# ChicyChen/LOCO-Edit

Measured on AMD Instinct MI355X. Metric: edit-directions/sec (top-5 PMP-Jacobian SVD @256^2) + vT cos-sim vs ref, higher is better.
Workload: dtype bf16x3 (split-bf16 MFMA operands, fp32 accumulate + fp32 storage); 1 GPU; CelebA-HQ DDPM 256x256 top-5 local basis (l_eye-sized mask, L=2400), t=0.6T, 12 power iterations, one GPU; multi_gpu_form=single, probes_total=5, probes_per_gpu=5, kept=5, n_iter=12, mask_L=2400, weights=synthetic seed 0, streams=2

## Files before the change

loco-edit_amd/csrc/conv_bf16_kernel.h:

```cpp
#pragma once
#include "kernels.h"
#include <cstdlib>
#include <type_traits>

namespace loco {


typedef float f32x16 __attribute__((ext_vector_type(16)));
typedef float f32x4 __attribute__((ext_vector_type(4)));
typedef f32x4 f32x4_u __attribute__((aligned(4)));
typedef float f32x2 __attribute__((ext_vector_type(2)));
typedef f32x2 f32x2_u __attribute__((aligned(4)));
typedef __bf16 bf16x8 __attribute__((ext_vector_type(8)));
typedef _Float16 f16x8 __attribute__((ext_vector_type(8)));
typedef short s16x8 __attribute__((ext_vector_type(8)));

enum : int { PR_BF16X3 = 0, PR_F16 = 1 };

constexpr int BKC = 16;
constexpr bool LIVE_MASK = true;
constexpr bool EARLY_W = true;
constexpr int NDUMMY = 8;

__device__ __forceinline__ float sigmoidf2_(float y) { return __builtin_amdgcn_rcpf(1.0f + __expf(-y)); }
// ... 608 lines not shown
            have = hi < nsg4 * nhy2 && sg < nseg && hy < halo_h;
            if (!have) v_q4 = 0;
        } else if (tid < 4 * per_q) {
            int rem;
            idivmod_small(tid, per_q, v_q4, rem);
            idivmod_small(rem, nseg, hy, sg);
            have = true;
        }
        if (have) {
            int Y = oy0 - a.pad + hy, X0 = ox0 - a.pad + 4 * sg;
            bool rowok = (Y >= 0 && Y < a.Hin);
            v_pos0 = hy * halo_w + 4 * sg;
            v_cnt = halo_w - 4 * sg < 4 ? halo_w - 4 * sg : 4;
            v_voff = rowok ? Y * a.Win + X0 : 0;
#pragma unroll
            for (int pxi = 0; pxi < 4; ++pxi)
                if (rowok && X0 + pxi >= 0 && X0 + pxi < a.Win && pxi < v_cnt) v_pm |= 1u << pxi;
        }
#pragma unroll
        for (int pxi = 0; pxi < 4; ++pxi)
            v_rec[pxi] = (v_pos0 >= 0 && pxi < v_cnt) ? v_pos0 + pxi : halo_sz + (tid & (NDUMMY - 1));
        v_goff = (unsigned)(((long)v_q4 * 4 * in_plane + v_voff + 16) * 4);
    }

    int hoff[TN];
#pragma unroll
    for (int j = 0; j < TN; ++j) {
        int p = (wn * TN + j) * 32 + l31;
        int ty, tx;
        idivmod_small(p, TW, ty, tx);
        hoff[j] = ty * S * halo_w + tx * S;
    }
    int hbyte[TN];
#pragma unroll
    for (int j = 0; j < TN; ++j) hbyte[j] = hrec_off<PR>(hoff[j], khalf);
    int aoff_hi[TM], aoff_lo[TM];
#pragma unroll
    for (int i = 0; i < TM; ++i) {
        int p = (wm * TM + i) * 32 + l31;
        aoff_hi[i] = rec_off<PR>(p, khalf);
        aoff_lo[i] = PR == PR_F16 ? 0 : rec_off<PR>(p, 2 + khalf);
    }

    if constexpr (PHASE != 2) {
#pragma unroll
        for (int i = 0; i < TM; ++i)
#pragma unroll
            for (int j = 0; j < TN; ++j)
#pragma unroll
                for (int r = 0; r < 16; ++r) acc[i][j][r] = 0.0f;
    }

    const int nchunks = (a.Cin + BKC - 1) / BKC;
    const int cps = __builtin_amdgcn_readfirstlane((nchunks + a.nsplit - 1) / a.nsplit);
    const int cbeg = split * cps;
    const int cend = (cbeg + cps < nchunks) ? cbeg + cps : nchunks;

    const float* inb = a.in + (long)b * a.in_bs;
    const float2* sxb = NEEDP ? a.sx : nullptr;
    const float* scb = (MODE == CM_GN_SILU || MODE == CM_GN || MODE == CM_GN_GELU) ? a.sc + (long)b * a.scsh_bs : nullptr;
    const float* shb = (MODE == CM_GN_SILU || MODE == CM_GN || MODE == CM_GN_GELU) ? a.sh + (long)b * a.scsh_bs : nullptr;
    const int wpitch = (a.Cout + 31) & ~31;
    const uint4* wg = reinterpret_cast<const uint4*>(a.wb);

    float hv[NITEM][8];
    float2 pv[NEEDP ? NITEM : 1][8];
    float cA[(MODE == CM_NONE) ? 1 : 16], cB[(MODE == CM_NONE) ? 1 : 16];
    const float* tcb = NEEDP ? a.tc + (long)b * a.tc_bs : nullptr;

    constexpr int NPART = (!GEN && NROW >= 2) ? 2 : 1;
    constexpr int KP = 4 / NPART;
    struct HaloRegs {
        f32x4 dq[GEN ? 1 : KP];
        f32x4 sq[(!GEN && NEEDP) ? KP : 1][2];
        f32x4 cq[(!GEN && MODE != CM_NONE) ? (KP == 4 ? 2 : 1) : 1];
    };
    auto cq_a = [&](const HaloRegs& R, int kk) -> float {
        if constexpr (GEN || MODE == CM_NONE) return 0.f;
        else if constexpr (NEEDP) { if constexpr (KP == 4) return R.cq[kk >> 1][(kk & 1) * 2]; else return R.cq[0][kk * 2]; }
        else return R.cq[0][kk];
    };
    auto cq_b = [&](const HaloRegs& R, int kk) -> float {
        if constexpr (GEN || MODE == CM_NONE) return 0.f;
        else if constexpr (NEEDP) { if constexpr (KP == 4) return R.cq[kk >> 1][(kk & 1) * 2 + 1]; else return R.cq[0][kk * 2 + 1]; }
        else if constexpr (KP == 4) return R.cq[1][kk];
        else return R.cq[0][2 + kk];
    };
    HaloRegs hr;
    bool pf_live = true, dma_live = true;
#ifdef LOCO_DUAL_STAMP
    const bool wi_halo = (a.no_deep & 2) != 0, wi_dma = (a.no_deep & 4) != 0, wi_novalu = (a.no_deep & 8) != 0;
#endif
    auto prefetch_hv = [&](HaloRegs& R, int chunk, int part) {
        const unsigned cb = (unsigned)chunk * ((unsigned)(BKC * 4) * (unsigned)in_plane);
        const char* pk = reinterpret_cast<const char*>(inb - 16) + cb;
        const char* sk = reinterpret_cast<const char*>(reinterpret_cast<const float*>(sxb) - 32) + 2u * cb;
        const unsigned pl = (unsigned)in_plane * 4u;
#pragma unroll
        for (int kk = 0; kk < KP; ++kk) {
#ifdef LOCO_DUAL_STAMP
            const unsigned po = (pf_live && !wi_halo) ? v_goff + (unsigned)(part * KP + kk) * pl : 64u;
#else
            const unsigned po = pf_live ? v_goff + (unsigned)(part * KP + kk) * pl : 64u;
#endif
            R.dq[kk] = *reinterpret_cast<const f32x4_u*>(pk + po);
            if constexpr (NEEDP) {
                R.sq[kk][0] = *reinterpret_cast<const f32x4_u*>(sk + 2u * po);
                R.sq[kk][1] = *reinterpret_cast<const f32x4_u*>(sk + 2u * po + 16);
            }
        }
        const int c0 = chunk * BKC + v_q4 * 4 + part * KP;
        if constexpr (MODE != CM_NONE) {
            if constexpr (NEEDP) {
                R.cq[0] = *reinterpret_cast<const f32x4_u*>(tcb + 2 * c0);
                if constexpr (KP == 4) R.cq[1] = *reinterpret_cast<const f32x4_u*>(tcb + 2 * c0 + 4);
            } else if constexpr (KP == 4) {
                R.cq[0] = *reinterpret_cast<const f32x4_u*>(scb + c0);
                R.cq[1] = *reinterpret_cast<const f32x4_u*>(shb + c0);
// ... 9 lines not shown
#endif
        const int oct = v_q4 >> 1, half = v_q4 & 1;
#pragma unroll
        for (int pxi = 0; pxi < 4; ++pxi) {
            float r[KP];
#pragma unroll
            for (int kk = 0; kk < KP; ++kk) {
                float d = R.dq[kk][pxi];
                float v = d;
                if constexpr (MODE == CM_GN_SILU) {
                    float y = fmaf(cq_a(R, kk), d, cq_b(R, kk));
                    v = y * sigmoidf2_(y);
                } else if constexpr (MODE == CM_GN_GELU) {
                    v = act_fwd(fmaf(cq_a(R, kk), d, cq_b(R, kk)), ACT_GELU);
                } else if constexpr (MODE == CM_GN) {
                    v = fmaf(cq_a(R, kk), d, cq_b(R, kk));
                } else if constexpr (NEEDP) {
                    const float Sv = R.sq[kk][pxi >> 1][(pxi & 1) * 2], xh = R.sq[kk][pxi >> 1][(pxi & 1) * 2 + 1];
                    if constexpr (MODE == CM_TAN_SILU) v = Sv * fmaf(-xh, cq_b(R, kk), d - cq_a(R, kk));
                    else v = fmaf(-xh, cq_b(R, kk), fmaf(Sv, d, -cq_a(R, kk)));
                }
                r[kk] = ((v_pm >> pxi) & 1u) ? v : 0.0f;
            }
            unsigned char* dst = Hs + hrec_off<PR>(v_rec[pxi], oct) + half * 8 + part * (KP * 2);
            if constexpr (KP == 4) {
                uint2 h, l;
                cvt2<PR>(r[0], r[1], h.x, l.x);
                cvt2<PR>(r[2], r[3], h.y, l.y);
                *reinterpret_cast<uint2*>(dst) = h;
                if constexpr (PR == PR_BF16X3) *reinterpret_cast<uint2*>(dst + 32) = l;
            } else {
                unsigned h, l;
                cvt2<PR>(r[0], r[1], h, l);
                *reinterpret_cast<unsigned*>(dst) = h;
                if constexpr (PR == PR_BF16X3) *reinterpret_cast<unsigned*>(dst + 32) = l;
            }
        }
    };
    auto load_consts = [&](int chunk) {
        const int c0 = chunk * BKC;
        if constexpr (MODE != CM_NONE) {
#pragma unroll
            for (int kk = 0; kk < 16; ++kk) {
                int c = c0 + kk < a.Cin ? c0 + kk : a.Cin - 1;
                if constexpr (NEEDP) { cA[kk] = tcb[2 * c]; cB[kk] = tcb[2 * c + 1]; }
                else { cA[kk] = scb[c]; cB[kk] = shb[c]; }
            }
        }
    };
    auto load_regs = [&](float (&hvd)[NITEM][8], int chunk) {
        int c0 = chunk * BKC;
        long poff = 0;
        if constexpr (PIN) {
            const int cpp = a.Cin >> 6, ph = __builtin_amdgcn_readfirstlane(idiv_small(chunk, cpp));
            c0 = (chunk - ph * cpp) * BKC;
            poff = (long)(ph >> 1) * 2 * a.Win + (ph & 1);
        }
        if (PIN || c0 + BKC <= a.Cin) {
            if constexpr (TAPS == 9 && !NEEDP) {
                const unsigned lm = pf_live ? 0xffffffffu : 0u;
                const long pb4 = in_plane * 4;
                const unsigned char* pk = reinterpret_cast<const unsigned char*>(inb) + (long)c0 * pb4;
#pragma unroll
                for (int k = 0; k < 8; ++k) {
#pragma unroll
                    for (int i = 0; i < NITEM; ++i) hvd[i][k] = *reinterpret_cast<const float*>(pk + ((ivoff[i] * 4u) & lm));
                    pk += pb4;
                }
            } else {
#pragma unroll
            for (int k = 0; k < 8; ++k) {
                const float* pk = inb + (long)(c0 + k) * in_plane + poff;
                const float2* sk = NEEDP ? sxb + (long)(c0 + k) * in_plane : nullptr;
#pragma unroll
                for (int i = 0; i < NITEM; ++i) {
                    hvd[i][k] = pk[pf_live ? ivoff[i] : 0u];
                    if constexpr (NEEDP) pv[i][k] = sk[pf_live ? ivoff[i] : 0u];
                }
            }
            }
        } else {
#pragma unroll
            for (int i = 0; i < NITEM; ++i) {
#pragma unroll
                for (int k = 0; k < 8; ++k) {
                    int c = c0 + ioct[i] * 8 + k;
                    int cc = c < a.Cin ? c : a.Cin - 1;
                    unsigned vo = ivoff[i] - (unsigned)(ioct[i] * 8 * (int)in_plane);
                    float v = inb[(long)cc * in_plane + vo];
                    hvd[i][k] = c < a.Cin ? v : 0.0f;
                    if constexpr (NEEDP) {
                        float2 pp = sxb[(long)cc * in_plane + vo];
                        pv[i][k] = c < a.Cin ? pp : make_float2(0.f, 0.f);
                    }
                }
            }
        }
    };
    auto prefetch_h = [&](int chunk, int part) {
        if constexpr (!GEN) { prefetch_hv(hr, chunk, part); return; }
        load_consts(chunk);
        load_regs(hv, chunk);
    };
    unsigned wrel[NWV];
#pragma unroll
    for (int i = 0; i < NWV; ++i) {
        int e = tid + i * NTHR;
        if (e >= WTOT) e = WTOT - 1;
        int tap = e / (MT * NPC), rem = e - tap * (MT * NPC);
        int rec = co0 + rem / NPC;
        if (rec >= wpitch) rec = wpitch - 1;
        wrel[i] = (unsigned)((tap * wpitch + rec) * NPC + (rem % NPC)) * 16u;
    }
    typedef __attribute__((address_space(3))) unsigned char lds_u8;
    typedef const __attribute__((address_space(1))) unsigned char glb_u8;
    auto dma_w = [&](int chunk, int row, unsigned char* Wdst) {
        const unsigned char* wbase = reinterpret_cast<const unsigned char*>(wg) +
                                     (unsigned)(chunk * TAPS + row * NTS) * ((unsigned)wpitch * (unsigned)RB);
#pragma unroll
        for (int i = 0; i < NWV; ++i) {
            const int e0 = (wave * 64 + i * NTHR);
            if ((WTOT % NTHR) == 0 || e0 < WTOT)
#ifdef LOCO_DUAL_STAMP
                __builtin_amdgcn_global_load_lds((glb_u8*)(wbase + ((dma_live && !wi_dma) ? wrel[i] : 0u)), (lds_u8*)(Wdst + e0 * 16), 16, 0, 0);
#else
                __builtin_amdgcn_global_load_lds((glb_u8*)(wbase + (dma_live ? wrel[i] : 0u)), (lds_u8*)(Wdst + e0 * 16), 16, 0, 0);
#endif
        }
    };
    auto stage_regs = [&](const float (&hvs)[NITEM][8], int chunk, unsigned char* Hd, auto whole_tag) {
        constexpr bool WHOLE = decltype(whole_tag)::value;
        const int c0 = chunk * BKC;
#pragma unroll
        for (int i = 0; i < NITEM; ++i) {
            if (ipos[i] < 0) continue;
            float v[8];
#pragma unroll
            for (int k = 0; k < 8; ++k) {
                int c = c0 + ioct[i] * 8 + k;
                float r = 0.0f;
                if (ival[i] && (WHOLE || c < a.Cin)) {
                    float d = hvs[i][k];
                    if constexpr (MODE == CM_NONE) {
                        r = d;
                    } else {
                        const float ca = ioct[i] ? cA[8 + k] : cA[k];
                        const float cb = ioct[i] ? cB[8 + k] : cB[k];
                        if constexpr (MODE == CM_GN_SILU) {
                            float y = fmaf(ca, d, cb);
                            r = y * sigmoidf2_(y);
                        } else if constexpr (MODE == CM_GN_GELU) {
                            r = act_fwd(fmaf(ca, d, cb), ACT_GELU);
                        } else if constexpr (MODE == CM_GN) {
                            r = fmaf(ca, d, cb);
                        } else {
                            float Sv = pv[i][k].x, xh = pv[i][k].y;
                            if constexpr (MODE == CM_TAN_SILU) r = Sv * fmaf(-xh, cb, d - ca);
                            else r = fmaf(-xh, cb, fmaf(Sv, d, -ca));
                        }
                    }
                }
                v[k] = r;
            }
            uint4 hi, lo;
            split8<PR>(v, hi, lo);
            *reinterpret_cast<uint4*>(Hd + hrec_off<PR>(ipos[i], ioct[i])) = hi;
            if constexpr (PR == PR_BF16X3) *reinterpret_cast<uint4*>(Hd + hrec_off<PR>(ipos[i], 2 + ioct[i])) = lo;
        }
    };
    auto stage_h = [&](int chunk, int part) {
        if constexpr (!GEN) { stage_hv(hr, part); return; }
        stage_regs(hv, chunk, Hs, std::false_type{});
    };

    constexpr int NLO = PR == PR_BF16X3 ? 1 : 0;
    struct Frag { s16x8 ah[TM], al[NLO ? TM : 1], bh[TN], bl[NLO ? TN : 1]; };
    auto load_frag = [&](Frag& f, int row, int tp) {
        const int tapoff = (TAPS == 9) ? row * halo_w + tp : (TAPS == 4 ? tap0 + row * halo_w + tp : 0);
#pragma unroll
        for (int i = 0; i < TM; ++i) {
            f.ah[i] = *reinterpret_cast<const s16x8*>(Ws + tp * MT * RB + aoff_hi[i]);
#if defined(LOCO_WI_NOLO)
            if constexpr (NLO) f.al[i] = f.ah[i];
#else
            if constexpr (NLO) f.al[i] = *reinterpret_cast<const s16x8*>(Ws + tp * MT * RB + aoff_lo[i]);
#endif
        }
#pragma unroll
        for (int j = 0; j < TN; ++j) {
            const unsigned char* hp = Hs + tapoff * HP + hbyte[j];
            f.bh[j] = *reinterpret_cast<const s16x8*>(hp);
#if defined(LOCO_WI_NOLO)
            if constexpr (NLO) f.bl[j] = f.bh[j];
#else
            if constexpr (NLO) f.bl[j] = *reinterpret_cast<const s16x8*>(hp + 32);
#endif
        }
    };
    auto mma_frag = [&](const Frag& f) {
#pragma unroll
        for (int i = 0; i < TM; ++i)
#pragma unroll
            for (int j = 0; j < TN; ++j) {
                if constexpr (PR == PR_F16) {
                    acc[i][j] = __builtin_amdgcn_mfma_f32_32x32x16_f16(__builtin_bit_cast(f16x8, f.ah[i]),
                                                                       __builtin_bit_cast(f16x8, f.bh[j]), acc[i][j], 0, 0, 0);
                } else {
                    const bf16x8 ah = __builtin_bit_cast(bf16x8, f.ah[i]), al = __builtin_bit_cast(bf16x8, f.al[i]);
                    const bf16x8 bh = __builtin_bit_cast(bf16x8, f.bh[j]), bl = __builtin_bit_cast(bf16x8, f.bl[j]);
                    acc[i][j] = __builtin_amdgcn_mfma_f32_32x32x16_bf16(al, bh, acc[i][j], 0, 0, 0);
                    acc[i][j] = __builtin_amdgcn_mfma_f32_32x32x16_bf16(ah, bl, acc[i][j], 0, 0, 0);
                    acc[i][j] = __builtin_amdgcn_mfma_f32_32x32x16_bf16(ah, bh, acc[i][j], 0, 0, 0);
                }
            }
    };

    auto mma_one = [&](const Frag& f, int i, int j) {
        if constexpr (PR == PR_F16) {
            acc[i][j] = __builtin_amdgcn_mfma_f32_32x32x16_f16(__builtin_bit_cast(f16x8, f.ah[i]),
                                                               __builtin_bit_cast(f16x8, f.bh[j]), acc[i][j], 0, 0, 0);
        } else {
            const bf16x8 ah = __builtin_bit_cast(bf16x8, f.ah[i]), al = __builtin_bit_cast(bf16x8, f.al[i]);
            const bf16x8 bh = __builtin_bit_cast(bf16x8, f.bh[j]), bl = __builtin_bit_cast(bf16x8, f.bl[j]);
#if defined(LOCO_WI_MFMA16)
// ... 188 lines not shown
            issue(S3{}, cbeg + 3);
            commit(S0{}, cbeg, Hsb, Wsb);
            issue(S0{}, cbeg + 4);
            stage_end();
        }
        auto body = [&](auto stag, const int ci) {
            const int chunk = cbeg + ci;
            unsigned char* const Wcur = Wsb + (ci & 1) * WBYTES;
            unsigned char* const Wnxt = Wsb + ((ci + 1) & 1) * WBYTES;
            unsigned char* const Hcur = Hsb + (ci & 1) * HBYTES;
            unsigned char* const Hnxt = Hsb + ((ci + 1) & 1) * HBYTES;
            Ws = Wcur; Hs = Hcur;
            Frag f0;
            load_frag(f0, 0, 0);
            __builtin_amdgcn_sched_barrier(0);
            mma_frag(f0);
            commit(stag, cclamp(chunk + 1), Hnxt, Wnxt);
            issue(stag, chunk + 1 + D);
            stage_end();
        };
        int ci = 0;
        for (; ci + D <= nch; ci += D) {
            body(S1{}, ci); body(S2{}, ci + 1); body(S3{}, ci + 2); body(S0{}, ci + 3);
        }
        if (ci < nch) body(S1{}, ci);
        if (ci + 1 < nch) body(S2{}, ci + 1);
        if (ci + 2 < nch) body(S3{}, ci + 2);
      }
    }
    if (!deep_done) {
    if (nch > 0) {
        dma_w(cbeg, 0, Wsb);
        Hs = Hsb;
        if constexpr (!GEN && NPART == 2) {
            HaloRegs hr2;
            prefetch_hv(hr, cbeg, 0);
            prefetch_hv(hr2, cbeg, 1);
            stage_hv(hr, 0);
            stage_hv(hr2, 1);
        } else {
#pragma unroll
            for (int part = 0; part < NPART; ++part) {
                prefetch_h(cbeg, part);
                stage_h(cbeg, part);
            }
        }
        asm volatile("s_waitcnt vmcnt(0)" ::: "memory");
        if (NROW == 1 || NPART == 2) prefetch_h(cclamp(cbeg + 1), 0);
        stage_end();
    }
    for (int ci = 0; ci < nch; ++ci) {
        const int chunk = cbeg + ci;
        if constexpr (PIN) {
            const int ph = __builtin_amdgcn_readfirstlane(idiv_small(chunk, a.Cin >> 6));
            tap0 = (1 - (ph >> 1)) * halo_w + 1 - (ph & 1);
        }
#pragma unroll
        for (int row = 0; row < NROW; ++row) {
            const int s_ = ci * NROW + row;
            unsigned char* const Wcur = Wsb + (s_ & 1) * WBYTES;
            unsigned char* const Wnxt = Wsb + ((s_ + 1) & 1) * WBYTES;
            unsigned char* const Hcur = Hsb + (ci & 1) * HBYTES;
            unsigned char* const Hnxt = Hsb + ((ci + 1) & 1) * HBYTES;
            constexpr bool one = (NROW == 1);
            const int st_part = one ? 0 : (NPART == 2 ? (row == 0 ? 0 : row == 1 ? 1 : -1) : (row == NROW - 1 ? 0 : -1));
            const int ld_part = one ? 0 : (NPART == 2 ? (row == 0 ? 1 : row == 1 ? 0 : -1) : (row == 0 ? 0 : -1));
            const int ld_chunk = one ? chunk + 2 : ((NPART == 2 && row == 1) ? chunk + 2 : chunk + 1);
            constexpr bool MIDLOAD = !GEN;
            constexpr int NLD = KP + (NEEDP ? 2 * KP + 1 : (MODE != CM_NONE ? 2 : 0));
            {
                const int r1 = (row + 1) % NROW, dc = (row + 1) / NROW;
                dma_live = LIVE_MASK ? (chunk + dc <= clast) : true;
                dma_w(cclamp(chunk + dc), r1, Wnxt);
                dma_live = true;
            }
            Ws = Wcur; Hs = Hcur;
            Frag f0, f1;
            load_frag(f0, row, 0);
            if (NTS > 1) load_frag(f1, row, 1);
            __builtin_amdgcn_sched_barrier(0);
            mma_frag(f0);
            __builtin_amdgcn_sched_barrier(0);
            if (NTS > 2) load_frag(f0, row, 2);
            __builtin_amdgcn_sched_barrier(0);
            if (NTS > 1) mma_frag(f1);
            if (st_part >= 0) { Hs = Hnxt; stage_h(cclamp(chunk + 1), st_part); Hs = Hcur; }
            if (MIDLOAD && ld_part >= 0) { pf_live = LIVE_MASK ? (ld_chunk <= clast) : true; prefetch_h(cclamp(ld_chunk), ld_part); pf_live = true; }
            if (NTS > 2) mma_frag(f0);
            __builtin_amdgcn_sched_barrier(0);
            if (MIDLOAD && ld_part >= 0) {
                asm volatile("s_waitcnt vmcnt(%0)" :: "n"(NLD) : "memory");
            } else {
                asm volatile("s_waitcnt vmcnt(0)" ::: "memory");
                if (!MIDLOAD && ld_part >= 0) { pf_live = LIVE_MASK ? (ld_chunk <= clast) : true; prefetch_h(cclamp(ld_chunk), ld_part); pf_live = true; }
            }
            stage_end();
        }
    }
    }

    }

    if constexpr (PHASE == 1) {
        asm volatile("s_waitcnt lgkmcnt(0)" ::: "memory");
        __builtin_amdgcn_s_barrier();
        return;
    }
    LP_STAMP(3);
    if constexpr (POLY) conv_lowp_epilogue_poly<WM, WN, TM, TN>(a, acc, smem_b, cot_id, pa_, oy0, ox0, TW, tile_id, b);
    else conv_lowp_epilogue<WM, WN, TM, TN, (TAPS == 1 && PHASE == 0) ? (EPI_COT1 | EPI_STATS) : EPI_STATS>(a, acc, smem_b, co0, oy0, ox0, TW, tile_id, b, split);
    LP_STAMP(4);
#undef LP_STAMP
}

constexpr int lowp_min_waves(int taps, int nthr) { return (taps == 1 && nthr <= 256) ? 2 : 1; }
template <int TAPS, int WM, int WN, int TM, int TN, int MODE, int STG>
__global__ __launch_bounds__(WM * WN * 64, lowp_min_waves(TAPS, WM * WN * 64)) void conv_mfma_bf16x3(ConvArgs a) {
    f32x16 acc[TM][TN];
    conv_lowp_body<PR_BF16X3, TAPS, WM, WN, TM, TN, MODE, STG>(a, acc);
}
// ... 34 lines not shown
    if (lds > 64 * 1024) {
        static DeviceOnce once;
        if (first_on_device(once)) {
            (void)hipFuncSetAttribute(reinterpret_cast<const void*>(kern), hipFuncAttributeMaxDynamicSharedMemorySize,
                                      160 * 1024);
        }
    }
    hipLaunchKernelGGL(kern, grid, dim3(WM * WN * 64), lds, st, a);
}

template <int PR, int TAPS, int WM, int WN, int TM, int TN, int MODE>
static void launch_one_b(const ConvArgs& a, hipStream_t st) {
    const bool general = a.stride != 1 || a.upsample || a.zins || (a.Cin % BKC) != 0 || !a.in_padded;
    if constexpr (MODE == CM_NONE) {
        if (a.stride == 2) launch_one_b2<PR, TAPS, WM, WN, TM, TN, MODE, 2>(a, st);
        else if (TAPS == 9 && !general) launch_one_b2<PR, TAPS, WM, WN, TM, TN, MODE, 0>(a, st);
        else launch_one_b2<PR, TAPS, WM, WN, TM, TN, MODE, 1>(a, st);
        return;
    }
    if constexpr (MODE == CM_GN_SILU || MODE == CM_TAN_SILU || MODE == CM_GN_GELU) {
        if (general) { launch_one_b2<PR, TAPS, WM, WN, TM, TN, MODE, 1>(a, st); return; }
    }
    launch_one_b2<PR, TAPS, WM, WN, TM, TN, MODE, 0>(a, st);
}


template <int PR, int MODE>
void launch_kcat_b(const ConvArgs& a, hipStream_t st) {
    constexpr int WM = 2, WN = 4, TM = 2, TN = 2, MT = 128, NT = 256;
    const int TW = a.Wout < 32 ? a.Wout : 32, TH = NT / TW;
    size_t lds = (size_t)3 * 3 * MT * rec_bytes<PR>() + 2 * ((size_t)(TW + 2) * (TH + 2) + NDUMMY) * halo_pitch<PR>();
    dim3 grid(((a.Hout * a.Wout) / NT) * ((a.Cout + MT - 1) / MT) * a.B * a.nsplit);
    void (*kern)(ConvArgs);
    if constexpr (PR == PR_F16) kern = &conv_kcat_f16<WM, WN, TM, TN, MODE>;
    else kern = &conv_kcat_bf16x3<WM, WN, TM, TN, MODE>;
    static DeviceOnce once;
    if (first_on_device(once))
        (void)hipFuncSetAttribute(reinterpret_cast<const void*>(kern), hipFuncAttributeMaxDynamicSharedMemorySize, 160 * 1024);
    hipLaunchKernelGGL(kern, grid, dim3(WM * WN * 64), lds, st, a);
}

template <int PR>
void launch_poly_b(const ConvArgs& a, hipStream_t st) {
    ConvArgs v = a;
    v.Cout = 4 * a.Cout; v.Hout = a.Hin; v.Wout = a.Win;
    v.upsample = 0; v.zins = 0; v.stride = 1; v.pad = 1; v.nsplit = 1;
    launch_one_b2<PR, 4, 2, 4, 2, 2, CM_NONE, 0>(v, st);
}

template <int PR>
void launch_poly_in_b(const ConvArgs& a, hipStream_t st) {
    ConvArgs v = a;
    v.Cin = 4 * a.Cin; v.Hin = a.Hin / 2; v.Win = a.Win / 2;
    v.upsample = 0; v.zins = 0; v.stride = 1; v.pad = 1; v.nsplit = 1;
    launch_one_b2<PR, 4, 2, 4, 2, 2, CM_NONE, 1>(v, st);
}

template <int PR, int TAPS, int MODE>
void launch_tile_b(const ConvArgs& a, hipStream_t st) {
    switch (a.tile) {
        case 5:
            launch_one_b<PR, TAPS, 2, 4, 2, 2, MODE>(a, st);
            break;
        case 0: launch_one_b<PR, TAPS, 2, 2, 2, 2, MODE>(a, st); break;
        case 1: launch_one_b<PR, TAPS, 4, 1, 1, 2, MODE>(a, st); break;
        case 2: launch_one_b<PR, TAPS, 1, 4, 1, 1, MODE>(a, st); break;
        default: launch_one_b<PR, TAPS, 2, 2, 1, 1, MODE>(a, st); break;
    }
}


}
```

loco-edit_amd/csrc/conv_plan.hip:

```cpp
#include "kernels.h"
#include <cstdio>
#include <cstdlib>

namespace loco {

constexpr int BKC = 16;
constexpr int BKF = 8;

static const int kMT[6] = {128, 128, 32, 64, 128, 128}, kNT[6] = {128, 64, 128, 64, 256, 256};

static int env_int(const char* name, int dflt) {
    const char* e = getenv(name);
    return e ? atoi(e) : dflt;
}
static int pick_tile(int Cout, int HW) {
    if (HW >= 128) return Cout > 32 ? 0 : 2;
    return Cout > 64 ? 1 : 3;
}

static int conv_pick_nsplit(int Cin, int Cout, int Hout, int Wout, int B) {
    const int t = pick_tile(Cout, Hout * Wout);
    long blocks = (long)((Hout * Wout) / kNT[t]) * ((Cout + kMT[t] - 1) / kMT[t]) * B;
    int nchunks = (Cin + BKF - 1) / BKF;
    if (blocks >= 384 || nchunks < 8) return 1;
    int want = (int)((512 + blocks - 1) / blocks);
    int maxs = nchunks / 4;
    if (want > maxs) want = maxs;
    if (want > 32) want = 32;
    return want < 1 ? 1 : want;
}

static int conv_bf16_pick_tile(int Cout, int HW, int B, int tile_override) {
    if (B <= 1 && HW <= 1024 && HW >= 64 && (Cout % 64) == 0) return 3;
    int t = pick_tile(Cout, HW);
    if (t == 0 && HW >= 256) {
        if (tile_override >= 0) return tile_override;
        return 5;
    }
    return t;
}

constexpr int kTile0MaxHW = 65536;

static int bf16_tile_of(const ConvArgs& a, int tile_override = -1) {
    int tile = conv_bf16_pick_tile(a.Cout, a.Hout * a.Wout, a.B, tile_override);
    if (tile == 4) tile = 5;
    if (tile == 5 && a.taps == 1 && !a.gemm && a.B >= 2 && a.Hout * a.Wout <= kTile0MaxHW) return 0;
    if (a.stride == 2 && tile == 5) tile = 0;
    return tile;
}
static int tile_for(const ConvArgs& a, int prec, int tile_override) {
    return prec ? bf16_tile_of(a, tile_override) : pick_tile(a.Cout, a.Hout * a.Wout);
}
static int conv_bf16_tile_pixels(const ConvArgs& a) { return a.poly == 1 ? 512 : a.gemm ? 256 : kNT[a.tile]; }
int conv_bf16_tile_couts(const ConvArgs& a) { return a.gemm ? 64 * a.gemm_tm : kMT[a.tile]; }

static bool conv_poly_ok(const ConvEnv& e, const ConvArgs& a, int taps) {
    static const bool on = env_int("LOCO_POLYPHASE", 1) != 0;
    if (!on || e.prec < 1 || taps != 9 || a.mode != CM_NONE || !(a.upsample || a.zins) || a.stride != 1) return false;
    if (!(e.prec == 2 ? a.wph : a.wpb) || !a.in_padded || a.res || a.Cin2 > 0 || a.cot_d) return false;
    if (a.upsample ? a.pad != 1 : (a.pad != 1 && a.pad != 2)) return false;
    if ((a.Cin % BKC) != 0 || (a.Cout % 128) != 0 || a.B < 2) return false;
    if (a.Hin * a.Win < 4096 || a.Win < 32 || (a.Win % 32) != 0 || (a.Hin % 8) != 0) return false;
    return a.Hout == 2 * a.Hin && a.Wout == 2 * a.Win;
}
static bool conv_poly_in_ok(const ConvEnv& e, const ConvArgs& a, int taps) {
    static const bool on = env_int("LOCO_POLYPHASE", 1) != 0;
    if (!on || e.prec < 1 || taps != 9 || a.mode != CM_NONE || !a.pool2 || a.upsample || a.zins || a.stride != 1 || a.pad != 1) return false;
    if (!(e.prec == 2 ? a.wqh : a.wqb) || a.res || a.bias2 || a.Cin2 > 0 || a.cot_d) return false;
    if ((a.Cin % BKC) != 0 || (a.Cout % 128) != 0 || a.B < 2 || ((a.Hin | a.Win) & 1)) return false;
    if (a.Hout * a.Wout < 4096 || a.Wout < 32 || (a.Wout % 32) != 0 || (a.Hout % 8) != 0) return false;
    return a.Hin == 2 * a.Hout && a.Win == 2 * a.Wout;
}

static int conv_bf16_pick_nsplit(int Cin, int Cout, int Hout, int Wout, int B, int chip_share, int taps, int lanes) {
    const int HW = Hout * Wout;
    int t = conv_bf16_pick_tile(Cout, HW, B, -1);
    if (t == 4) t = 5;
    if (taps == 1 && t == 5 && B >= 2 && HW <= kTile0MaxHW) t = 0;
    long blocks = (long)(HW / kNT[t]) * ((Cout + kMT[t] - 1) / kMT[t]) * B;
    int nchunks = (Cin + BKC - 1) / BKC;
    int target = chip_share > 1 ? 256 / chip_share : (lanes == 2 ? 240 : 256);
    if (target < 32) target = 32;
    if (blocks >= target / 2 || nchunks < 8) return 1;
    int want = (int)(target / blocks);
    int maxs = nchunks / 4;
    if (want > maxs) want = maxs;
    if (want > 32) want = 32;
    return want < 1 ? 1 : want;
}

static bool conv_lowp_can_kcat(const ConvArgs& a) {
    static const bool on = env_int("LOCO_KCAT", 1) != 0;
    return on && a.Cin2 > 0 && a.nsplit == 1 && bf16_tile_of(a) == 5 && a.stride == 1 && !a.upsample && !a.zins && a.pad == 1 &&
           (a.Cin % BKC) == 0 && (a.Cin2 % BKC) == 0 && a.in_padded &&
           (a.mode == CM_GN_SILU || a.mode == CM_GN_GELU || a.mode == CM_TAN_SILU);
}
static bool conv_lowp_can_fuse_stats(const ConvArgs& a) {
    return a.nsplit <= 1 && !a.gemm && (a.Cout % conv_bf16_tile_couts(a)) == 0;
}

static bool conv_pair_ok(const ConvArgs& a) {
    static const bool on = env_int("LOCO_CONV_PAIR", 1) != 0;
    if (!on || a.poly || a.Hout * a.Wout < 16384 || a.taps != 9 || a.Cin2 > 0 || a.nsplit != 1 || a.stride != 1 || a.upsample || a.zins ||
        a.pad != 1 || !a.in_padded || (a.Cin % (2 * BKC)) != 0 || (a.Cout % 128) != 0 || (a.Wout % 32) != 0 || (a.Hout % 8) != 0)
        return false;
    if (!(a.mode == CM_NONE || a.mode == CM_GN_SILU || a.mode == CM_TAN_SILU || a.mode == CM_COT_SILU)) return false;
    return a.tile == 5;
}

static ConvArgs conv_shift_batch(const ConvArgs& a, int nb) {
    ConvArgs t = a;
    t.B = a.B - nb;
    t.in += (long)nb * a.in_bs; t.out += (long)nb * a.out_bs;
    if (t.prim) t.prim += (long)nb * a.prim_bs;
    if (t.bias2) t.bias2 += (long)nb * a.bias2_bs;
    if (t.res) t.res += (long)nb * a.res_bs;
    if (t.sc) { t.sc += (long)nb * a.scsh_bs; t.sh += (long)nb * a.scsh_bs; }
    if (t.mr) t.mr += (long)nb * a.mr_bs;
    if (t.tst) t.tst += (long)nb * a.tst_bs;
    if (t.tc) t.tc += (long)nb * a.tc_bs;
    if (t.in2) t.in2 += (long)nb * a.in2_bs;
    if (t.cot_d) { t.cot_d += (long)nb * a.cot_d_bs; t.cot_tc += (long)nb * a.cot_tc_bs; }
    if (t.st_part) t.st_part += (long)nb * a.Cout * ((a.Hout * a.Wout) / conv_bf16_tile_pixels(a)) * 2;
// ... 54 lines not shown
    while (s > 1 && nchunks / s < 4) --s;
    const size_t one = (size_t)(r / per_probe) * a.Cout * a.Hout * a.Wout;
    while (s > 1 && (size_t)s * one > partial_floats) --s;
    *split = s;
    return s > 1 ? (int)(r / per_probe) : 0;
}

static int stats_route(const ConvEnv& e, const StatAsk* q, bool want, ConvArgs& x, int s0, int B, int* keep_ntile) {
    if (!q || q->kind == ST_NONE) return SR_NONE;
    const int alone = q->norm ? SR_ALONE : SR_NONE;
    if (!want) return alone;
    if (x.nsplit > 1) return !q->norm ? SR_NONE : ((x.Hout * x.Wout) % 4 == 0 ? SR_SPLITK : SR_ALONE);
    const int ntile = (x.Hout * x.Wout) / conv_bf16_tile_pixels(x);
    const size_t need = (size_t)x.B * x.Cout * ntile * 2;
    const int epi = q->norm ? SR_EPI : SR_KEEP;
    const bool kept = q->keep && s0 == 0 && x.B == B && need <= q->keep_floats;
    if (q->kind == ST_FWD && x.poly != 1 && conv_lowp_can_fuse_stats(x) && (kept || (q->norm && need <= e.stpart_floats))) {
        x.st_part = kept ? q->keep : e.stpart; x.st_kind = ST_FWD;
        if (kept) *keep_ntile = ntile;
        return epi;
    }
    const bool cot_cache = q->kind == ST_COT && q->norm && q->sx && x.poly != 1;
    if ((q->kind == ST_TAN || cot_cache) && e.fuse_lin && !x.cot_d && conv_lowp_can_fuse_stats(x)) {
        const size_t lane_off = (size_t)e.lane_s0 * (q->keep_floats / e.max_batch);
        const bool keptl = q->kind == ST_TAN && q->keep && s0 == 0 && x.B == B && lane_off + need <= q->keep_floats;
        if (keptl || (q->norm && need <= e.stpart_floats)) {
            x.st_part = keptl ? q->keep + lane_off : e.stpart; x.st_kind = q->kind; x.st_x = q->prim;
            if (q->kind == ST_COT) x.st_sx = q->sx;
            if (keptl) *keep_ntile = ntile;
            return epi;
        }
    }
    return alone;
}

static ConvLaunch plan_launch(const ConvEnv& e, const StatAsk* q, bool want, const ConvArgs& x, int s0, int B, int* keep_ntile) {
    ConvLaunch l;
    l.args = x;
    l.s0 = s0;
    l.args.tile = tile_for(x, e.prec, -1);
    l.stats = stats_route(e, q, want, l.args, s0, B, keep_ntile);
    if (l.stats == SR_EPI || l.stats == SR_KEEP) l.ntile = (x.Hout * x.Wout) / conv_bf16_tile_pixels(l.args);
    conv_plan_tile_pair(l.args, e.prec, -1);
    return l;
}

ConvPlan plan_conv(const ConvEnv& e, const ConvArgs& a0, int taps, const StatAsk* q, const ConvArgs* sc) {
    ConvPlan p;
    ConvArgs a = a0;
    a.taps = taps;
    a.gemm = 0;
    a.poly = 0;
    if (a.pool2) {
        if (conv_poly_in_ok(e, a, taps)) a.poly = 2;
        else {
            p.pool_after = true; p.pool_out = a.out; p.pool_out_bs = a.out_bs; p.pool_acc = a.accumulate;
            a.out = a.pool_tmp; a.out_bs = a.pool_tmp_bs; a.Hout = a.Hin; a.Wout = a.Win; a.accumulate = 0; a.pool2 = 0;
        }
    }
    if (sc) {
        ConvArgs t = a;
        t.nsplit = e.prec >= 1 ? conv_bf16_pick_nsplit(a.Cin, a.Cout, a.Hout, a.Wout, a.B, e.chip_share, 9, e.lanes) : 2;
        t.in2 = sc->in; t.in2_bs = sc->in_bs; t.Cin2 = sc->Cin;
        const long per_probe = (long)((a.Hout * a.Wout) / 256) * ((a.Cout + 127) / 128);
        if (e.prec >= 1 && taps == 9 && !short_tail(per_probe, a.B) && !a.bias2 && conv_lowp_can_kcat(t)) {
            a.in2 = sc->in; a.in2_bs = sc->in_bs; a.Cin2 = sc->Cin; a.in2_padded = sc->in_padded;
            a.wb2 = e.prec == 2 ? sc->wh : sc->wb;
            a.bias2 = sc->bias; a.bias2_bs = 0;
            a.res = nullptr;
        } else {
            p.sc_first = true;
            a.res = sc->out; a.res_bs = sc->out_bs;
        }
    }
    if (e.prec == 2) a.wb = a.wh;
    a.no_deep = e.deep1 ? 0 : 1;
    a.nsplit = e.prec >= 1 ? conv_bf16_pick_nsplit(a.Cin, a.Cout, a.Hout, a.Wout, a.B, e.chip_share, taps, e.lanes)
                           : conv_pick_nsplit(a.Cin, a.Cout, a.Hout, a.Wout, a.B);
    if (a.cot_d) {
        ConvArgs t = a;
        t.tile = bf16_tile_of(t);
        const long per_probe = (long)((a.Hout * a.Wout) / conv_bf16_tile_pixels(t)) * ((a.Cout + 127) / 128);
        p.cot = e.prec >= 1 && taps == 1 && a.nsplit == 1 && !short_tail(per_probe, a.B) && conv_lowp_can_fuse_stats(t);
        if (!p.cot) { a.cot_d = nullptr; a.cot_d_bs = 0; a.cot_sx = nullptr; a.cot_tc = nullptr; a.cot_tc_bs = 0; }
    }
    while (a.nsplit > 1 && (size_t)a.nsplit * a.B * a.Cout * a.Hout * a.Wout > e.partial_floats) a.nsplit >>= 1;
    if (a.nsplit < 1) a.nsplit = 1;
    a.partial = e.partial;
    a.partial_floats = e.partial_floats;
    if (!a.poly && conv_poly_ok(e, a, taps)) a.poly = 1;
    if (a.poly == 1) { a.nsplit = 1; a.wb = e.prec == 2 ? a.wph : a.wpb; }
    if (a.poly == 2) { a.nsplit = 1; a.wb = e.prec == 2 ? a.wqh : a.wqb; }
    conv_plan_family(a, e.prec);
    a.tile = tile_for(a, e.prec, -1);
    int split = 1;
    const int tail = e.prec >= 1 && a.nsplit == 1 && a.B >= 2 && !a.gemm && !a.poly ? tail_split(a, e.partial_floats, &split) : 0;
    const bool want = q && q->kind != ST_NONE && e.prec >= 1 && e.fuse_stats;
    if (!tail) {
        p.l[0] = plan_launch(e, q, want, a, 0, a.B, &p.keep_ntile);
        return p;
    }
    const bool per_part = want && q->norm && (q->kind == ST_FWD || (e.fuse_lin && (a.Hout * a.Wout) % 4 == 0));
    p.stats_all = !per_part && q && q->kind != ST_NONE && q->norm;
    const StatAsk* ql = per_part ? q : nullptr;
    const int nb = a.B - tail;
    ConvArgs m = a, t = conv_shift_batch(a, nb);
    m.B = nb;
    t.nsplit = split;
    p.nl = 2;
    p.l[0] = plan_launch(e, ql, want, m, 0, a.B, &p.keep_ntile);
    p.l[1] = plan_launch(e, ql, want, t, nb, a.B, &p.keep_ntile);
    return p;
}

void polyphase_fold(int kind, int nin, int nout, const float* w, long so, long si, long st, float* out) {
    static const int sel[3][2][2][3] = {
        {{{1, 0, 0}, {0, 1, 1}}, {{1, 1, 0}, {0, 0, 1}}},
        {{{1, 0, 0}, {0, 0, 1}}, {{0, 1, 0}, {0, 0, 0}}},
        {{{0, 0, 0}, {0, 1, 0}}, {{1, 0, 0}, {0, 0, 1}}}};
    const long V = 4L * nout;
    for (int i = 0; i < nin; ++i)
        for (int pa = 0; pa < 2; ++pa)
            for (int pb = 0; pb < 2; ++pb)
                for (int ty = 0; ty < 2; ++ty)
                    for (int tx = 0; tx < 2; ++tx)
                        for (int o = 0; o < nout; ++o) {
                            double acc = 0.0;
                            for (int ky = 0; ky < 3; ++ky)
                                for (int kx = 0; kx < 3; ++kx)
                                    if (sel[kind][pa][ty][ky] && sel[kind][pb][tx][kx]) acc += (double)w[o * so + i * si + (3 * ky + kx) * st];
                            out[((long)i * 4 + 2 * ty + tx) * V + polyphase_vcout(nout, pa, pb, o)] = (float)acc;
                        }
}

void polyphase_fold_in(int nin, int nout, const float* w, long so, long si, long st, float* out, int noutP) {
    for (int p = 0; p < 2; ++p)
        for (int q = 0; q < 2; ++q)
            for (int i = 0; i < nin; ++i)
                for (int ty = 0; ty < 2; ++ty)
                    for (int tx = 0; tx < 2; ++tx) {
                        const int m = 2 * ty + 1 - p, n = 2 * tx + 1 - q;
                        for (int o = 0; o < nout; ++o) {
                            double acc = 0.0;
                            for (int a = 0; a < 2; ++a)
                                for (int b = 0; b < 2; ++b) {
// ... 41 lines not shown
```

loco-edit_amd/csrc/engine.hip:

```cpp
#include <hip/hip_runtime.h>

#include <algorithm>
#include <array>
#include <cmath>
#include <cstdio>
#include <cstdlib>
#include <cstring>
#include <map>
#include <memory>
#include <thread>
#include <atomic>
#include <string>
#include <vector>

#include "../../include/loco_hip.h"
#ifdef LOCO_DIAG
#include "../../include/loco_hip_diag.h"
#endif
#include "kernels.h"
#include "program.h"
#ifdef LOCO_DIAG
#include "conv_plan_text.h"
#endif

// ... 2351 lines not shown
    const long in_e = (long)cin * ((geom && geom != 4) ? HW / 4 : HW), out_e = (long)cout * HW;
    if ((in_e + out_e + (geom == 4 ? out_e / 4 : 0)) * B > (long)c->cfg.max_batch * c->prog->per_sample || 2 * in_e > (long)c->prog->per_sample ||
        in_e > c->prog->sx_total) { c->err = "bench_conv: shape exceeds the arenas"; return -2; }
    float* in = c->arenaT;
    float* out = c->arenaT + in_e * B;
    const int bz = getenv("LOCO_BENCH_ZERO") ? atoi(getenv("LOCO_BENCH_ZERO")) : 0;
    const float zs = (bz & 1) ? 0.0f : 1.0f, zw = (bz & 2) ? 0.0f : 1.0f;
    launch_fill_random(in, in_e * B, 1u, zs, st);
    launch_fill_random(c->arenaP, in_e, 2u, zs, st);
    launch_fill_random(reinterpret_cast<float*>(c->sxcache), 2 * in_e, 3u, zs, st);
    launch_fill_random(c->statsP, c->prog->stats_per_sample, 4u, 1.0f, st);
    launch_fill_random(c->statsT, c->prog->stats_per_sample * B, 5u, 0.01f, st);
    size_t wfl = (size_t)((cin + 15) / 16) * 16 * (geom ? 16 : taps) * ((cout + 31) & ~31);
    if (wfl * 2 > c->partial_floats) { c->err = "bench_conv: weights exceed workspace"; return -2; }
    float* wf = c->partial + c->partial_floats - wfl * 2;
    launch_fill_random(wf, (long)wfl * 2, 6u, 0.05f * zw, st);
    if (c->prec == 1) {
        const long nrec = (long)((cin + 15) / 16) * (geom ? 16 : taps) * ((cout + 31) & ~31);
        hipLaunchKernelGGL(diag_fill_records, dim3((unsigned)((nrec + 255) / 256)), dim3(256), 0, st,
                           reinterpret_cast<unsigned char*>(wf), nrec, (cout + 31) & ~31, 7u, 0.05f * zw);
    }
    ConvArgs a; conv_defaults(a);
    a.in = in; a.in_bs = in_e; a.Cin = cin; a.Hin = H; a.Win = W;
    a.prim = c->arenaP; a.prim_bs = 0; a.sx = c->sxcache;
    a.w = wf; a.wb = wf; a.wh = wf;
    a.out = out; a.out_bs = out_e; a.Cout = cout; a.Hout = H; a.Wout = W; a.B = B;
    a.mode = mode; a.pad = taps == 9 ? 1 : 0; a.in_padded = 1; a.taps = taps;
    if (geom == 4) {
        a.pool2 = 1; a.pool_tmp = out; a.pool_tmp_bs = out_e;
        a.out = out + out_e * B; a.out_bs = out_e / 4; a.Hout = H / 2; a.Wout = W / 2;
        a.wqb = wf; a.wqh = wf;
    } else if (geom) {
        a.Hin = H / 2; a.Win = W / 2;
        if (geom == 1) a.upsample = 1; else { a.zins = 1; a.pad = geom == 2 ? 2 : 1; }
        a.wpb = wf; a.wph = wf;
    }
    a.sc = c->statsP; a.sh = c->statsP + cin; a.scsh_bs = 0; a.mr = c->statsP + 2 * cin; a.mr_bs = 0;
    a.gamma_ = c->statsP; a.tst = c->statsT; a.tst_bs = c->prog->stats_per_sample; a.cpg = cin / c->cfg.gn_groups;
    a.tc = c->statsT + 64; a.tc_bs = c->prog->stats_per_sample;
    if (a.cpg < 1) a.cpg = 1;
    a.nsplit = 1; a.partial = c->partial;
    a.partial_floats = c->partial_floats - wfl * 2;
    if (getenv("LOCO_BENCH_COT") && atoi(getenv("LOCO_BENCH_COT")) && taps == 1) {
        if ((in_e + 2 * out_e) * B > (long)c->cfg.max_batch * c->prog->per_sample || out_e > c->prog->sx_total ||
            2L * cout > c->prog->stats_per_sample) { c->err = "bench_conv: cot operands exceed the arenas"; return -2; }
        launch_fill_random(out + out_e * B, out_e * B, 8u, zs, st);
        if (out_e > in_e) launch_fill_random(reinterpret_cast<float*>(c->sxcache), 2 * out_e, 3u, zs, st);
        a.cot_d = out + out_e * B; a.cot_d_bs = out_e; a.cot_sx = c->sxcache; a.cot_tc = c->statsT; a.cot_tc_bs = c->prog->stats_per_sample;
    }
    if (getenv("LOCO_BENCH_ACC") && atoi(getenv("LOCO_BENCH_ACC"))) a.accumulate = 1;
    conv_plan_family(a, c->prec);
    if (const char* e = getenv("LOCO_DUAL_WHATIF")) a.no_deep = atoi(e);
    conv_plan_tile_pair(a, c->prec, tile);
    if (geom) {
        ConvEnv e;
        e.prec = c->prec; e.partial = a.partial; e.partial_floats = a.partial_floats; e.max_batch = c->cfg.max_batch;
        a.poly = plan_conv(e, a, taps, nullptr, nullptr).l[0].args.poly;
        if (a.poly) a.nsplit = 1;
        if (geom == 4 && a.poly != 2) { c->err = "bench_conv: the shape does not take the pooled polyphase launch"; return -2; }
    }
    auto run = [&]() {
        if (c->prec == 1) launch_conv_bf16x3(a, taps, st);
        else if (c->prec == 2) launch_conv_f16(a, taps, st);
        else launch_conv(a, taps, st);
        launch_conv_splitk_reduce(a, st);
    };
    run();
    HIPCHK(c, hipEventRecord(c->ev0, st));
    for (int i = 0; i < iters; ++i) run();
    HIPCHK(c, hipEventRecord(c->ev1, st));
    HIPCHK(c, hipEventSynchronize(c->ev1));
    c->bench_out = out; c->bench_out_count = (int64_t)out_e * B;
    float ms = 0.f;
    HIPCHK(c, hipEventElapsedTime(&ms, c->ev0, c->ev1));
    *ms_avg = ms / iters;
    HIPCHK(c, hipGetLastError());
    return 0;
}

}
__global__ void diag_scale_tc(const float* tc, const float* mr, int C, int cpg, long n, int by_rstd, float* out) {
    const long i = (long)blockIdx.x * 256 + threadIdx.x;
    if (i >= n) return;
    const float f = by_rstd ? mr[2 * (int)((i % C) / cpg) + 1] : 1.0f;
    out[2 * i] = f * tc[2 * i];
    out[2 * i + 1] = f * tc[2 * i + 1];
}
extern "C" {
int loco_debug_conv(loco_ctx* c, const loco_conv_desc* d, char* plan, int64_t cap, void* stream) {
    if (!c) return -2;
    if (!d || d->struct_size != (int32_t)sizeof(loco_conv_desc)) { c->err = "debug_conv: descriptor size mismatch"; return -2; }
    if (finalize_params(c)) return -3;
    hipStream_t st = (hipStream_t)stream;
    const int taps = d->taps, k = taps == 9 ? 3 : 1, B = d->B;
    if ((taps != 9 && taps != 1) || d->Cin < 1 || d->Cout < 1 || d->Hin < 1 || d->Win < 1 || B < 1 || (d->stride != 1 && d->stride != 2) ||
        d->mode < CM_NONE || d->mode > CM_GN_GELU || (d->upsample && d->zins) || (d->stride == 2 && (d->upsample || d->zins)) ||
        !d->weight || !d->in || !d->out) { c->err = "debug_conv: bad descriptor"; return -2; }
    if (d->stride == 2 && ((d->Hin | d->Win) & 1)) { c->err = "debug_conv: stride 2 needs an even map"; return -2; }
    const bool lin = d->mode == CM_TAN_SILU || d->mode == CM_COT_SILU;
    if (d->mode != CM_NONE && (!d->sc || !d->sh)) { c->err = "debug_conv: the prologue modes need sc / sh"; return -2; }
    if (lin && (!d->prim || !d->mr || !d->gamma || !d->tst || !d->tc || d->cpg < 1 || d->Cin % d->cpg)) {
        c->err = "debug_conv: modes 3 / 4 need prim, mr, gamma, tst, tc and cpg"; return -2;
    }
    if (d->Cin2 > 0 && (!d->in2 || !d->w2)) { c->err = "debug_conv: the second operator needs in2 and w2"; return -2; }
    if (d->Cin2 > 0 && (d->res || d->accumulate || taps != 9)) {
        c->err = "debug_conv: the second operator goes with a 3x3 conv without res / accumulate"; return -2;
    }
    if (d->cot_d && (!d->cot_prim || !d->cot_sc || !d->cot_sh || !d->cot_mr || !d->cot_tc || d->cot_cpg < 1 || d->Cout % d->cot_cpg)) {
        c->err = "debug_conv: the norm-cotangent term needs cot_prim, cot_sc, cot_sh, cot_mr, cot_tc and cot_cpg"; return -2;
    }
    if (d->pool2 && (taps != 9 || d->stride != 1 || d->upsample || d->zins || d->mode != CM_NONE || d->Cin2 > 0 || d->res || d->cot_d ||
                     ((d->Hin | d->Win) & 1))) { c->err = "debug_conv: pool2 goes with a raw 3x3 stride-1 conv of an even map"; return -2; }
    const int Hout = (d->stride == 2 || d->pool2) ? d->Hin / 2 : (d->upsample || d->zins) ? 2 * d->Hin : d->Hin;
    const int Wout = (d->stride == 2 || d->pool2) ? d->Win / 2 : (d->upsample || d->zins) ? 2 * d->Win : d->Win;
// ... 319 lines not shown
```

Before: 20.41 edit-directions/s.

## Pair polyphase chunks for vector input loads and enable split-K on small pooled convs

The pooled polyphase (poly=2) conv now orders chunks so that the two horizontally adjacent phases form consecutive chunk pairs. Both phases are fetched with one float2 load and the second is staged from registers, and the weight DMA chunk index is remapped to match. The planner also allows poly=2 on smaller outputs (16-wide tiles), picks a split-K factor rounded to even chunk counts when the output is under 4096 pixels, and skips poly for strided-conv cases and some accumulate shapes. A bench path that runs the whole plan is added. This trades extra registers for fewer global loads and more parallelism on small layers, at the risk of higher register pressure and a split-K reduce pass.

```diff
diff --git a/loco-edit_amd/csrc/conv_bf16_kernel.h b/loco-edit_amd/csrc/conv_bf16_kernel.h
--- a/loco-edit_amd/csrc/conv_bf16_kernel.h
+++ b/loco-edit_amd/csrc/conv_bf16_kernel.h
@@ -684,7 +684,7 @@
     }
 
     const int nchunks = (a.Cin + BKC - 1) / BKC;
-    const int cps = __builtin_amdgcn_readfirstlane((nchunks + a.nsplit - 1) / a.nsplit);
+    const int cps = __builtin_amdgcn_readfirstlane(((nchunks + a.nsplit - 1) / a.nsplit + (PIN ? 1 : 0)) & (PIN ? ~1 : ~0));
     const int cbeg = split * cps;
     const int cend = (cbeg + cps < nchunks) ? cbeg + cps : nchunks;
 
@@ -696,6 +696,7 @@
     const uint4* wg = reinterpret_cast<const uint4*>(a.wb);
 
     float hv[NITEM][8];
+    float hvq[PIN ? NITEM : 1][8];
     float2 pv[NEEDP ? NITEM : 1][8];
     float cA[(MODE == CM_NONE) ? 1 : 16], cB[(MODE == CM_NONE) ? 1 : 16];
     const float* tcb = NEEDP ? a.tc + (long)b * a.tc_bs : nullptr;
@@ -811,9 +812,9 @@
         int c0 = chunk * BKC;
         long poff = 0;
         if constexpr (PIN) {
-            const int cpp = a.Cin >> 6, ph = __builtin_amdgcn_readfirstlane(idiv_small(chunk, cpp));
-            c0 = (chunk - ph * cpp) * BKC;
-            poff = (long)(ph >> 1) * 2 * a.Win + (ph & 1);
+            const int cpp = a.Cin >> 6, hc = chunk >> 1, p = hc >= cpp ? 1 : 0;
+            c0 = (hc - p * cpp) * BKC;
+            poff = (long)p * 2 * a.Win;
         }
         if (PIN || c0 + BKC <= a.Cin) {
             if constexpr (TAPS == 9 && !NEEDP) {
@@ -833,7 +834,12 @@
                 const float2* sk = NEEDP ? sxb + (long)(c0 + k) * in_plane : nullptr;
 #pragma unroll
                 for (int i = 0; i < NITEM; ++i) {
-                    hvd[i][k] = pk[pf_live ? ivoff[i] : 0u];
+                    if constexpr (PIN) {
+                        const f32x2 v2 = *reinterpret_cast<const f32x2_u*>(pk + (pf_live ? ivoff[i] : 0u));
+                        hvd[i][k] = v2[0]; hvq[i][k] = v2[1];
+                    } else {
+                        hvd[i][k] = pk[pf_live ? ivoff[i] : 0u];
+                    }
                     if constexpr (NEEDP) pv[i][k] = sk[pf_live ? ivoff[i] : 0u];
                 }
             }
@@ -858,6 +864,7 @@
     };
     auto prefetch_h = [&](int chunk, int part) {
         if constexpr (!GEN) { prefetch_hv(hr, chunk, part); return; }
+        if constexpr (PIN) { if (chunk & 1) return; }
         load_consts(chunk);
         load_regs(hv, chunk);
     };
@@ -874,6 +881,10 @@
     typedef __attribute__((address_space(3))) unsigned char lds_u8;
     typedef const __attribute__((address_space(1))) unsigned char glb_u8;
     auto dma_w = [&](int chunk, int row, unsigned char* Wdst) {
+        if constexpr (PIN) {
+            const int cpp = a.Cin >> 6, hc = chunk >> 1, p = hc >= cpp ? 1 : 0;
+            chunk = (2 * p + (chunk & 1)) * cpp + hc - p * cpp;
+        }
         const unsigned char* wbase = reinterpret_cast<const unsigned char*>(wg) +
                                      (unsigned)(chunk * TAPS + row * NTS) * ((unsigned)wpitch * (unsigned)RB);
 #pragma unroll
@@ -929,6 +940,16 @@
     };
     auto stage_h = [&](int chunk, int part) {
         if constexpr (!GEN) { stage_hv(hr, part); return; }
+        if constexpr (PIN) {
+            const bool odd = (chunk & 1) != 0;
+            float hq[NITEM][8];
+#pragma unroll
+            for (int i = 0; i < NITEM; ++i)
+#pragma unroll
+                for (int k = 0; k < 8; ++k) hq[i][k] = odd ? hvq[i][k] : hv[i][k];
+            stage_regs(hq, chunk, Hs, std::true_type{});
+            return;
+        }
         stage_regs(hv, chunk, Hs, std::false_type{});
     };
 
@@ -1223,8 +1244,8 @@
     for (int ci = 0; ci < nch; ++ci) {
         const int chunk = cbeg + ci;
         if constexpr (PIN) {
-            const int ph = __builtin_amdgcn_readfirstlane(idiv_small(chunk, a.Cin >> 6));
-            tap0 = (1 - (ph >> 1)) * halo_w + 1 - (ph & 1);
+            const int p = (chunk >> 1) >= (a.Cin >> 6) ? 1 : 0;
+            tap0 = (1 - p) * halo_w + 1 - (chunk & 1);
         }
 #pragma unroll
         for (int row = 0; row < NROW; ++row) {
@@ -1235,8 +1256,8 @@
             unsigned char* const Hnxt = Hsb + ((ci + 1) & 1) * HBYTES;
             constexpr bool one = (NROW == 1);
             const int st_part = one ? 0 : (NPART == 2 ? (row == 0 ? 0 : row == 1 ? 1 : -1) : (row == NROW - 1 ? 0 : -1));
-            const int ld_part = one ? 0 : (NPART == 2 ? (row == 0 ? 1 : row == 1 ? 0 : -1) : (row == 0 ? 0 : -1));
-            const int ld_chunk = one ? chunk + 2 : ((NPART == 2 && row == 1) ? chunk + 2 : chunk + 1);
+            const int ld_part = one ? 0 : (NPART == 2 ? (row == 0 ? 1 : row == 1 ? 0 : -1) : (row == (PIN ? NROW - 1 : 0) ? 0 : -1));
+            const int ld_chunk = one ? chunk + 2 : (((NPART == 2 && row == 1) || PIN) ? chunk + 2 : chunk + 1);
             constexpr bool MIDLOAD = !GEN;
             constexpr int NLD = KP + (NEEDP ? 2 * KP + 1 : (MODE != CM_NONE ? 2 : 0));
             {
@@ -1377,7 +1398,7 @@
 void launch_poly_in_b(const ConvArgs& a, hipStream_t st) {
     ConvArgs v = a;
     v.Cin = 4 * a.Cin; v.Hin = a.Hin / 2; v.Win = a.Win / 2;
-    v.upsample = 0; v.zins = 0; v.stride = 1; v.pad = 1; v.nsplit = 1;
+    v.upsample = 0; v.zins = 0; v.stride = 1; v.pad = 1;
     launch_one_b2<PR, 4, 2, 4, 2, 2, CM_NONE, 1>(v, st);
 }
 
diff --git a/loco-edit_amd/csrc/conv_plan.hip b/loco-edit_amd/csrc/conv_plan.hip
--- a/loco-edit_amd/csrc/conv_plan.hip
+++ b/loco-edit_amd/csrc/conv_plan.hip
@@ -55,13 +55,19 @@
 static int conv_bf16_tile_pixels(const ConvArgs& a) { return a.poly == 1 ? 512 : a.gemm ? 256 : kNT[a.tile]; }
 int conv_bf16_tile_couts(const ConvArgs& a) { return a.gemm ? 64 * a.gemm_tm : kMT[a.tile]; }
 
+static bool poly_tiles_ok(int H, int W, int minw) {
+    static const int minw_env = env_int("LOCO_POLY_MINW", 0);
+    if (W < (minw_env > 0 ? minw_env : minw)) return false;
+    return W >= 32 ? ((W % 32) == 0 && (H % 8) == 0) : (W == 16 && (H % 16) == 0);
+}
 static bool conv_poly_ok(const ConvEnv& e, const ConvArgs& a, int taps) {
     static const bool on = env_int("LOCO_POLYPHASE", 1) != 0;
     if (!on || e.prec < 1 || taps != 9 || a.mode != CM_NONE || !(a.upsample || a.zins) || a.stride != 1) return false;
     if (!(e.prec == 2 ? a.wph : a.wpb) || !a.in_padded || a.res || a.Cin2 > 0 || a.cot_d) return false;
     if (a.upsample ? a.pad != 1 : (a.pad != 1 && a.pad != 2)) return false;
     if ((a.Cin % BKC) != 0 || (a.Cout % 128) != 0 || a.B < 2) return false;
-    if (a.Hin * a.Win < 4096 || a.Win < 32 || (a.Win % 32) != 0 || (a.Hin % 8) != 0) return false;
+    if (!poly_tiles_ok(a.Hin, a.Win, 32)) return false;
+    if (a.accumulate && a.B == 2 && a.Win < 64) return false;
     return a.Hout == 2 * a.Hin && a.Wout == 2 * a.Win;
 }
 static bool conv_poly_in_ok(const ConvEnv& e, const ConvArgs& a, int taps) {
@@ -69,7 +75,7 @@
     if (!on || e.prec < 1 || taps != 9 || a.mode != CM_NONE || !a.pool2 || a.upsample || a.zins || a.stride != 1 || a.pad != 1) return false;
     if (!(e.prec == 2 ? a.wqh : a.wqb) || a.res || a.bias2 || a.Cin2 > 0 || a.cot_d) return false;
     if ((a.Cin % BKC) != 0 || (a.Cout % 128) != 0 || a.B < 2 || ((a.Hin | a.Win) & 1)) return false;
-    if (a.Hout * a.Wout < 4096 || a.Wout < 32 || (a.Wout % 32) != 0 || (a.Hout % 8) != 0) return false;
+    if (!poly_tiles_ok(a.Hout, a.Wout, 16)) return false;
     return a.Hin == 2 * a.Hout && a.Win == 2 * a.Wout;
 }
 
@@ -230,7 +236,7 @@
     a.gemm = 0;
     a.poly = 0;
     if (a.pool2) {
-        if (conv_poly_in_ok(e, a, taps)) a.poly = 2;
+        if (!sc && conv_poly_in_ok(e, a, taps)) a.poly = 2;
         else {
             p.pool_after = true; p.pool_out = a.out; p.pool_out_bs = a.out_bs; p.pool_acc = a.accumulate;
             a.out = a.pool_tmp; a.out_bs = a.pool_tmp_bs; a.Hout = a.Hin; a.Wout = a.Win; a.accumulate = 0; a.pool2 = 0;
@@ -268,7 +274,13 @@
     a.partial_floats = e.partial_floats;
     if (!a.poly && conv_poly_ok(e, a, taps)) a.poly = 1;
     if (a.poly == 1) { a.nsplit = 1; a.wb = e.prec == 2 ? a.wph : a.wpb; }
-    if (a.poly == 2) { a.nsplit = 1; a.wb = e.prec == 2 ? a.wqh : a.wqb; }
+    if (a.poly == 2) {
+        a.nsplit = a.Hout * a.Wout < 4096 ? conv_bf16_pick_nsplit(4 * a.Cin, a.Cout, a.Hout, a.Wout, a.B, e.chip_share, taps, e.lanes) : 1;
+        while (a.nsplit > 1 && (size_t)a.nsplit * a.B * a.Cout * a.Hout * a.Wout > e.partial_floats) a.nsplit >>= 1;
+        const int nch = 4 * a.Cin / BKC;
+        while (a.nsplit > 1 && (((nch + a.nsplit - 1) / a.nsplit + 1) & ~1) * (a.nsplit - 1) >= nch) --a.nsplit;
+        a.wb = e.prec == 2 ? a.wqh : a.wqb;
+    }
     conv_plan_family(a, e.prec);
     a.tile = tile_for(a, e.prec, -1);
     int split = 1;
diff --git a/loco-edit_amd/csrc/engine.hip b/loco-edit_amd/csrc/engine.hip
--- a/loco-edit_amd/csrc/engine.hip
+++ b/loco-edit_amd/csrc/engine.hip
@@ -2427,14 +2427,31 @@
     conv_plan_family(a, c->prec);
     if (const char* e = getenv("LOCO_DUAL_WHATIF")) a.no_deep = atoi(e);
     conv_plan_tile_pair(a, c->prec, tile);
+    ConvPlan bench_plan;
+    bool whole_plan = false;
     if (geom) {
         ConvEnv e;
         e.prec = c->prec; e.partial = a.partial; e.partial_floats = a.partial_floats; e.max_batch = c->cfg.max_batch;
+        if (getenv("LOCO_BENCH_PLAN") && atoi(getenv("LOCO_BENCH_PLAN"))) {
+            e.lanes = getenv("LOCO_BENCH_LANES") ? atoi(getenv("LOCO_BENCH_LANES")) : 1;
+            bench_plan = plan_conv(e, a, taps, nullptr, nullptr);
+            whole_plan = true;
+        }
         a.poly = plan_conv(e, a, taps, nullptr, nullptr).l[0].args.poly;
         if (a.poly) a.nsplit = 1;
-        if (geom == 4 && a.poly != 2) { c->err = "bench_conv: the shape does not take the pooled polyphase launch"; return -2; }
+        if (geom == 4 && a.poly != 2 && !whole_plan) { c->err = "bench_conv: the shape does not take the pooled polyphase launch"; return -2; }
     }
     auto run = [&]() {
+        if (whole_plan) {
+            for (int li = 0; li < bench_plan.nl; ++li) {
+                const ConvArgs& x = bench_plan.l[li].args;
+                if (c->prec == 1) launch_conv_bf16x3(x, taps, st); else launch_conv_f16(x, taps, st);
+                if (x.nsplit > 1) launch_conv_splitk_reduce(x, st);
+            }
+            if (bench_plan.pool_after)
+                launch_pool2x2_sum(a.pool_tmp, a.pool_tmp_bs, bench_plan.pool_out, bench_plan.pool_out_bs, bench_plan.pool_acc, a.B, a.Cout, a.Hout, a.Wout, st);
+            return;
+        }
         if (c->prec == 1) launch_conv_bf16x3(a, taps, st);
         else if (c->prec == 2) launch_conv_f16(a, taps, st);
         else launch_conv(a, taps, st);
```

Result: no change. 20.61 edit-directions/s (median of 6 runs) (+1.0%).
